# qingxu-thu/INSR-PDE

Hardware: AMD Instinct MI355X
Metric: collocation-points/sec/timestep (incl. ∇/Δ residual + Adam) at 1/2/4/8 GPUs (higher is better)
Workload: dtype fp32

## Files before the change

insr-pde_amd/csrc/jet_x6.hpp:

```cpp
#pragma once
#include "jet_split.hpp"

namespace insr {

typedef short bf16x8 __attribute__((ext_vector_type(8)));
typedef unsigned u32x4 __attribute__((ext_vector_type(4)));
typedef unsigned u32x2 __attribute__((ext_vector_type(2)));
typedef __bf16 bf16x2v __attribute__((ext_vector_type(2)));

__device__ __forceinline__ unsigned pk_bf16(float a, float b) {
  const bf16x2v v = {(__bf16)a, (__bf16)b};
  return __builtin_bit_cast(unsigned, v);
}
__device__ __forceinline__ float bf_lo(unsigned p) { return __builtin_bit_cast(float, p << 16); }
__device__ __forceinline__ float bf_hi(unsigned p) { return __builtin_bit_cast(float, p & 0xffff0000u); }

__device__ __forceinline__ void split3(float a, float b, unsigned& h, unsigned& m, unsigned& l) {
  h = pk_bf16(a, b);
  float ra = a - bf_lo(h), rb = b - bf_hi(h);
  m = pk_bf16(ra, rb);
  ra -= bf_lo(m);
  rb -= bf_hi(m);
  l = pk_bf16(ra, rb);
}

template <int NQ>
constexpr int np_of() { return NQ == 4 ? 2 : NQ; }

template <int NQ>
struct FragQ {
  u32x4 q[np_of<NQ>()];
};

typedef _Float16 f16x2v __attribute__((ext_vector_type(2)));
typedef _Float16 f16x8 __attribute__((ext_vector_type(8)));
__device__ __forceinline__ unsigned pk_f16(float a, float b) {
  const f16x2v v = {(_Float16)a, (_Float16)b};
  return __builtin_bit_cast(unsigned, v);
}
using Frag3 = FragQ<3>;

template <int NQ>
__device__ __forceinline__ void splitq(float a, float b, unsigned (&o)[np_of<NQ>()]) {
  if constexpr (NQ == 4) {
    o[0] = pk_f16(a, b);
    const f16x2v h = __builtin_bit_cast(f16x2v, o[0]);
    o[1] = pk_f16(a - (float)h[0], b - (float)h[1]);
    return;
  }
  o[0] = pk_bf16(a, b);
  if constexpr (NQ > 1) {
    float ra = a - bf_lo(o[0]), rb = b - bf_hi(o[0]);
    o[1] = pk_bf16(ra, rb);
    if constexpr (NQ > 2) {
      ra -= bf_lo(o[1]);
      rb -= bf_hi(o[1]);
      o[2] = pk_bf16(ra, rb);
    }
  }
}

template <int NQ>
__device__ __forceinline__ FragQ<NQ> split_frag(const floatx4& v0, const floatx4& v1) {
  unsigned t[4][np_of<NQ>()];
  splitq<NQ>(v0[0], v0[1], t[0]);
  splitq<NQ>(v0[2], v0[3], t[1]);
  splitq<NQ>(v1[0], v1[1], t[2]);
  splitq<NQ>(v1[2], v1[3], t[3]);
  FragQ<NQ> f;
#pragma unroll
  for (int q = 0; q < np_of<NQ>(); ++q) f.q[q] = u32x4{t[0][q], t[1][q], t[2][q], t[3][q]};
  return f;
}

__device__ __forceinline__ floatx4 mfma_bf(const u32x4& a, const u32x4& b, floatx4 c) {
  return __builtin_amdgcn_mfma_f32_16x16x32_bf16(__builtin_bit_cast(bf16x8, a), __builtin_bit_cast(bf16x8, b), c,
                                                 0, 0, 0);
}

__device__ __forceinline__ floatx4 mfma_h(const u32x4& a, const u32x4& b, floatx4 c) {
  return __builtin_amdgcn_mfma_f32_16x16x32_f16(__builtin_bit_cast(f16x8, a), __builtin_bit_cast(f16x8, b), c, 0, 0, 0);
}

template <int NQ>
__device__ __forceinline__ floatx4 mfma_q(const FragQ<NQ>& a, const FragQ<NQ>& b, floatx4 c) {
  if constexpr (NQ == 4) {
    c = mfma_h(a.q[0], b.q[1], c);
    c = mfma_h(a.q[1], b.q[0], c);
    return mfma_h(a.q[0], b.q[0], c);
  }
  if constexpr (NQ == 3) {
    c = mfma_bf(a.q[1], b.q[1], c);
    c = mfma_bf(a.q[0], b.q[2], c);
    c = mfma_bf(a.q[2], b.q[0], c);
  }
  if constexpr (NQ >= 2) {
    c = mfma_bf(a.q[0], b.q[1], c);
    c = mfma_bf(a.q[1], b.q[0], c);
  }
  return mfma_bf(a.q[0], b.q[0], c);
}

template <int NQ, int PLANE>
__device__ __forceinline__ FragQ<NQ> lds_frag(const unsigned short* p) {
  FragQ<NQ> f;
#pragma unroll
  for (int q = 0; q < np_of<NQ>(); ++q) f.q[q] = *reinterpret_cast<const u32x4*>(p + q * PLANE);
  return f;
}

template <int NQ, int PLANE>
__device__ __forceinline__ void lds_put4(unsigned short* p, float a0, float a1, float a2, float a3) {
  unsigned u0[np_of<NQ>()], u1[np_of<NQ>()];
  splitq<NQ>(a0, a1, u0);
  splitq<NQ>(a2, a3, u1);
#pragma unroll
  for (int q = 0; q < np_of<NQ>(); ++q) *reinterpret_cast<u32x2*>(p + q * PLANE) = u32x2{u0[q], u1[q]};
}

template <int NT>
struct X6Geo {
  static constexpr int W = 16 * NT;
  static constexpr int WV = NT < 8 ? NT : 8;
  static constexpr int RPW = NT / WV;
  static constexpr int KC = NT / 2;
  static constexpr int LDB = W + 8;
  static constexpr int PLANE = 16 * LDB;
  static constexpr int THREADS = 64 * WV;
};

template <int NQ, int NT, int S, int T>
constexpr size_t fwd_x6_lds_bytes() {
  using G = X6Geo<NT>;
  const size_t planes = (size_t)T * S * np_of<NQ>() * G::PLANE * 2 + (NQ == 4 ? (2 * T * 8 + 2 + 8) * sizeof(float) : 0);
  const size_t red = (size_t)G::WV * T * S * 3 * 16 * sizeof(float);
  return planes > red ? planes : red;
}

__device__ __forceinline__ const u32x4* wsp_base(const float* prm, int din, int dout, int L, int W) {
  return reinterpret_cast<const u32x4*>(prm + wsplit_offset(din, dout, L, W));
}
template <int NQ, int NT>
__device__ __forceinline__ FragQ<NQ> wsp_frag(const u32x4* __restrict__ wsp, int L, int o, int j, int rt, int kc,
                                              int lane) {
  constexpr int W = 16 * NT, KC = NT / 2;
  if constexpr (NQ == 4) {
    const u32x4* p = wsp + 2 * wsplit_orient_vecs(L, W) + o * wsplit_f16_vecs(L, W) +
                     ((((long)(j - 1) * NT + rt) * KC + kc) * 2) * 64 + lane;
    FragQ<NQ> f;
    f.q[0] = p[0];
    f.q[1] = p[64];
    return f;
  }
  const u32x4* p = wsp + o * wsplit_orient_vecs(L, W) + ((((long)(j - 1) * NT + rt) * KC + kc) * 3) * 64 + lane;
  FragQ<NQ> f;
#pragma unroll
  for (int q = 0; q < NQ; ++q) f.q[q] = p[q * 64];
  return f;
}

__device__ __forceinline__ int f16_exp_for(float m) {
  if (!(m > 0.f && m <= 3.0e38f)) return 0;
  int k;
  (void)frexpf(m, &k);
  return min(max(15 - k, -100), 100);
}

__device__ __forceinline__ void block_tiles(int b, int N, int T, int nbal, int& tile0, int& cnt) {
  if (nbal > 0) {
    const long tiles = (N + 15) / 16;
    tile0 = (int)(((long)b * tiles) / nbal);
    cnt = (int)((((long)b + 1) * tiles) / nbal) - tile0;
  } else {
    const int tiles = (N + 15) / 16;
    tile0 = b * T;
    cnt = tiles - tile0 < T ? tiles - tile0 : T;
  }
}

template <int NQ, int NT, int S, bool LAP, int T>
__device__ __forceinline__ void fwd_x6_block(const float* __restrict__ x, int N, int din, int dout, int L,
                                             const float* __restrict__ prm, float* __restrict__ y,
                                             float* __restrict__ dy, float* __restrict__ lap,
                                             float* __restrict__ act, const int tile0, const int cnt_rt) {
  using G = X6Geo<NT>;
  constexpr int W = G::W, RPW = G::RPW, LDB = G::LDB, WV = G::WV, PLANE = G::PLANE, KC = G::KC;
  constexpr int NTAN = LAP ? S - 2 : S - 1;
  const int cnt = (T == 3 || T == 5) ? cnt_rt : T;
  extern __shared__ __attribute__((aligned(16))) float lds_f[];
  unsigned short* lds = reinterpret_cast<unsigned short*>(lds_f);
  const int wave = threadIdx.x >> 6, lane = threadIdx.x & 63, g = lane >> 4, c = lane & 15;
  const int ntiles = ((N + 63) / 64) * 4;
  const int rt0 = wave * RPW;
  const u32x4* wsp = wsp_base(prm, din, dout, L, W);
  float* zmx = lds_f + (T * S * np_of<NQ>() * PLANE) / 2;
  float usl[T];
#pragma unroll
  for (int t = 0; t < T; ++t) usl[t] = 1.f / kF16WScale;
  float ust = 1.f / kF16WScale;
  int* tflag = reinterpret_cast<int*>(zmx + 2 * T * 8);
  if constexpr (NQ == 4 && NTAN > 0) {
    if (threadIdx.x < 2) tflag[threadIdx.x] = 0;
  }

  float xv[T][3];
#pragma unroll
  for (int t = 0; t < T; ++t) {
    const int p = (tile0 + t) * 16 + c;
    for (int k = 0; k < 3; ++k) xv[t][k] = (t < cnt && p < N && k < din) ? x[(long)p * din + k] : 0.f;
  }

  floatx4 a[T][RPW][S];
  {
    const float* W0 = prm;
    const float* b0 = prm + (long)W * din;
#pragma unroll
    for (int i = 0; i < RPW; ++i) {
#pragma unroll
      for (int r = 0; r < 4; ++r) {
        const int n = 16 * (rt0 + i) + 4 * g + r;
        const float bn = b0[n];
        float w0[3] = {0.f, 0.f, 0.f};
        for (int k = 0; k < din; ++k) w0[k] = W0[n * din + k];
#pragma unroll
        for (int t = 0; t < T; ++t) {
          float z = bn;
          for (int k = 0; k < din; ++k) z = fmaf(w0[k], xv[t][k], z);
          a[t][i][0][r] = z;
#pragma unroll
          for (int k = 0; k < NTAN; ++k) a[t][i][1 + k][r] = w0[k];
          if constexpr (LAP) a[t][i][S - 1][r] = 0.f;
        }
      }
    }
  }
  for (int j = 0; j <= L; ++j) {
    if (j > 0) {
      const float* Wj = prm + hidden_off(din, W, j);
      const float* bj = Wj + (long)W * W;
#pragma unroll
      for (int i = 0; i < RPW; ++i) {
        const int rt = rt0 + i;
        FragQ<NQ> wf[KC];
#pragma unroll
        for (int kc = 0; kc < KC; ++kc) wf[kc] = wsp_frag<NQ, NT>(wsp, L, 0, j, rt, kc, lane);
        floatx4 bias = *reinterpret_cast<const floatx4*>(bj + 16 * rt + 4 * g);
        if constexpr (NQ == 4) bias *= kF16WScale;
#pragma unroll
        for (int t = 0; t < T; ++t) {
          a[t][i][0] = bias;
#pragma unroll
          for (int s = 1; s < S; ++s) a[t][i][s] = floatx4{0.f, 0.f, 0.f, 0.f};
        }
#pragma unroll
        for (int kc = 0; kc < KC; ++kc) {
#pragma unroll
          for (int t = 0; t < T; ++t) {
            if (t >= cnt) break;
#pragma unroll
            for (int s = 0; s < S; ++s) {
              const unsigned short* pb = lds + (t * S + s) * np_of<NQ>() * PLANE + c * LDB + 32 * kc + 8 * g;
              a[t][i][s] = mfma_q<NQ>(wf[kc], lds_frag<NQ, PLANE>(pb), a[t][i][s]);
            }
          }
        }
        if constexpr (NQ == 4) {
#pragma unroll
          for (int t = 0; t < T; ++t)
#pragma unroll
            for (int s = 0; s < S; ++s)
              a[t][i][s] *= (LAP && s == S - 1) ? usl[t] : (s > 0 ? ust : 1.f / kF16WScale);
        }
      }
    }
    if constexpr (NQ == 4 && LAP) {
      if (j < L) {
#pragma unroll
        for (int t = 0; t < T; ++t) {
          float mt = 0.f;
#pragma unroll
          for (int i = 0; i < RPW; ++i)
#pragma unroll
            for (int r = 0; r < 4; ++r) {
              float t2 = 0.f;
#pragma unroll
              for (int k = 0; k < NTAN; ++k) t2 = fmaf(a[t][i][1 + k][r], a[t][i][1 + k][r], t2);
              mt = fmaxf(mt, fmaf(OMEGA, fabsf(a[t][i][S - 1][r]), OMEGA2 * t2));
            }
          mt = wave_max(mt);
          if (lane == 0) zmx[((j & 1) * T + t) * 8 + wave] = mt;
        }
      }
    }
    auto tan_bound = [&]() -> float {
      float mt = 0.f;
      if (j == 0) {
        for (int n = lane; n < W; n += 64)
          for (int k = 0; k < NTAN; ++k) mt = fmaxf(mt, fabsf(prm[n * din + k]));
      } else {
#pragma unroll
        for (int t = 0; t < T; ++t)
#pragma unroll
          for (int i = 0; i < RPW; ++i)
#pragma unroll
            for (int k = 0; k < NTAN; ++k)
#pragma unroll
              for (int r = 0; r < 4; ++r) mt = fmaxf(mt, fabsf(a[t][i][1 + k][r]));
      }
      return OMEGA * mt;
    };
    bool tbig = false;
    if constexpr (NQ == 4 && NTAN > 0) {
      if (j < L) {
        tbig = __any(tan_bound() >= 32768.f);
        if (j > 0 && tbig && lane == 0) tflag[j & 1] = 1;
      }
    }
    if (j > 0 || (NQ == 4 && LAP)) __syncthreads();
    float sct = 1.f;
    if constexpr (NQ == 4 && NTAN > 0) {
      ust = 1.f / kF16WScale;
      if (j < L) {
        if (j > 0) tbig = __builtin_amdgcn_readfirstlane(tflag[j & 1]) != 0;
        if (tbig) {
          float mt = wave_max(tan_bound());
          if (j > 0) {
            float* tmx = reinterpret_cast<float*>(tflag + 2);
            if (lane == 0) tmx[wave] = mt;
            __syncthreads();
#pragma unroll
            for (int w = 0; w < WV; ++w) mt = fmaxf(mt, tmx[w]);
          }
          const int e = __builtin_amdgcn_readfirstlane(f16_exp_for(mt));
          sct = ldexpf(1.f, e);
          ust = ldexpf(1.f, -e) / kF16WScale;
        }
        if (j > 0 && threadIdx.x == 0) tflag[(j + 1) & 1] = 0;
      }
    }
    if (act) {
      const int ns = l0_rebuilt(j, L) ? 1 : S;
#pragma unroll
      for (int t = 0; t < T; ++t) {
        if (t >= cnt) break;
        float* base = act_base(act, j, ntiles, tile0 + t, S, NT);
#pragma unroll
        for (int i = 0; i < RPW; ++i)
#pragma unroll
          for (int s = 0; s < S; ++s)
            if (s < ns) *reinterpret_cast<floatx4*>(base + ((s * NT + rt0 + i) * 64 + lane) * 4) = a[t][i][s];
      }
    }
#pragma unroll
    for (int t = 0; t < T; ++t) sine_jet<RPW, S, LAP>(a[t]);
    if (j < L) {
      float sll[T];
#pragma unroll
      for (int t = 0; t < T; ++t) {
        sll[t] = 1.f;
        if constexpr (NQ == 4 && LAP) {
          float m = zmx[((j & 1) * T + t) * 8];
#pragma unroll
          for (int w = 1; w < WV; ++w) m = fmaxf(m, zmx[((j & 1) * T + t) * 8 + w]);
          const int e = f16_exp_for(m);
          sll[t] = ldexpf(1.f, e);
          usl[t] = ldexpf(1.f, -e) / kF16WScale;
        }
      }
#pragma unroll
      for (int t = 0; t < T; ++t)
#pragma unroll
        for (int i = 0; i < RPW; ++i)
#pragma unroll
          for (int s = 0; s < S; ++s) {
            unsigned short* pw = lds + (t * S + s) * np_of<NQ>() * PLANE + c * LDB + 16 * (rt0 + i) + 4 * g;
            const float sc = (LAP && s == S - 1) ? sll[t] : (s > 0 ? sct : 1.f);
            lds_put4<NQ, PLANE>(pw, sc * a[t][i][s][0], sc * a[t][i][s][1], sc * a[t][i][s][2], sc * a[t][i][s][3]);
          }
      __syncthreads();
    }
  }
  float* red = lds_f;
  const float* Wo = prm + out_off(din, W, L);
  const float* bo = Wo + (long)dout * W;
  for (int o = 0; o < dout; ++o) {
    float sv[T][S];
#pragma unroll
    for (int t = 0; t < T; ++t)
#pragma unroll
      for (int s = 0; s < S; ++s) sv[t][s] = 0.f;
#pragma unroll
    for (int i = 0; i < RPW; ++i) {
      const floatx4 w4 = *reinterpret_cast<const floatx4*>(Wo + (o * W + 16 * (rt0 + i) + 4 * g));
#pragma unroll
      for (int t = 0; t < T; ++t)
#pragma unroll
        for (int r = 0; r < 4; ++r)
#pragma unroll
          for (int s = 0; s < S; ++s) sv[t][s] = fmaf(w4[r], a[t][i][s][r], sv[t][s]);
    }
#pragma unroll
    for (int t = 0; t < T; ++t)
#pragma unroll
      for (int s = 0; s < S; ++s) {
        float v = sv[t][s];
        v += __shfl_xor(v, 16);
        v += __shfl_xor(v, 32);
        if (g == 0) red[(((wave * T + t) * S + s) * 3 + o) * 16 + c] = v;
      }
  }
  __syncthreads();
  static_assert(T <= 4 * WV, "output stage: one lane group per tile");
  if (wave * 4 + g < cnt) {
    const int t = wave * 4 + g;
    const int p = (tile0 + t) * 16 + c;
    if (p < N) {
      for (int o = 0; o < dout; ++o) {
        float tot[S];
#pragma unroll
        for (int s = 0; s < S; ++s) {
          tot[s] = 0.f;
#pragma unroll
          for (int w = 0; w < WV; ++w) tot[s] += red[(((w * T + t) * S + s) * 3 + o) * 16 + c];
        }
        y[(long)p * dout + o] = tot[0] + bo[o];
        if (dy)
          for (int k = 0; k < NTAN; ++k) dy[((long)p * dout + o) * din + k] = tot[1 + k];
        if constexpr (LAP) {
          if (lap) lap[(long)p * dout + o] = tot[S - 1];
        }
      }
    }
  }
}

template <int NQ, int NT, int S, bool LAP, int T>
constexpr int x6_fwd_min_waves() {
  return ((NT == 8 && (S == 1 || (S == 3 && T <= 2))) || (NQ == 4 && NT == 16 && S == 4 && !LAP && T == 1))
             ? 4
             : 1;
}

template <int NQ, int NT, int S, bool LAP, int T>
__global__ __launch_bounds__(X6Geo<NT>::THREADS, (x6_fwd_min_waves<NQ, NT, S, LAP, T>())) void jet_fwd_x6(
    const float* __restrict__ x, int N, int din, int dout, int L, const float* __restrict__ prm,
    float* __restrict__ y, float* __restrict__ dy, float* __restrict__ lap, float* __restrict__ act, int nbal) {
  int tile0, cnt;
  block_tiles(blockIdx.x, N, T, nbal, tile0, cnt);
  fwd_x6_block<NQ, NT, S, LAP, T>(x, N, din, dout, L, prm, y, dy, lap, act, tile0, cnt);
}

struct FwdJobsX6 {
  InsrJetJob job[kFwdJobs];
  int first[kFwdJobs + 1];
  int small[kFwdJobs];
  int nbal[kFwdJobs];
  int njobs;
};

template <int NQ, int NT, int S, bool LAP, int TA>
constexpr int x6_multi_min_waves() {
  return ((NT == 8 && (S == 1 || S == 3)) || (NQ == 4 && NT == 16 && S == 4 && !LAP && TA == 1)) ? 4 : 1;
}

template <int NQ, int NT, int S, bool LAP, int TA, int TB>
__global__ __launch_bounds__(X6Geo<NT>::THREADS, (x6_multi_min_waves<NQ, NT, S, LAP, TA>())) void jet_fwd_x6_multi(
    const FwdJobsX6 jobs, int din, int dout, int L) {
  const int b = blockIdx.x;
  int k = 0;
#pragma unroll
  for (int q = 1; q < kFwdJobs; ++q) k += (q < jobs.njobs && b >= jobs.first[q]) ? 1 : 0;
  const InsrJetJob& jb = jobs.job[k];
  const int dout_k = jb.d_out > 0 ? jb.d_out : dout;
  if constexpr (TA != TB) {
    if (jobs.small[k]) {
      fwd_x6_block<NQ, NT, S, LAP, TB>(jb.x, (int)jb.n, din, dout_k, L, jb.params, jb.y, jb.dy, jb.lap, jb.act,
                                       (b - jobs.first[k]) * TB, TB);
      return;
    }
  }
  int tile0, cnt;
  block_tiles(b - jobs.first[k], (int)jb.n, TA, jobs.nbal[k], tile0, cnt);
  fwd_x6_block<NQ, NT, S, LAP, TA>(jb.x, (int)jb.n, din, dout_k, L, jb.params, jb.y, jb.dy, jb.lap, jb.act, tile0, cnt);
}

struct FwdMixX6 {
  InsrJetJob job[kFwdJobs];
  int first[kFwdJobs + 1];
  int mode[kFwdJobs];
  float sc[kFwdJobs][3];
  int njobs;
};

constexpr int kMixV = 1, kMixG = 2, kMixL = 4, kMixA = 8;
#ifndef INSR_MIX_ADV_T
#define INSR_MIX_ADV_T 2
#endif
constexpr int kMixAdvT = INSR_MIX_ADV_T;

template <int NQ, int NT, int DIN, int BODIES>
constexpr size_t fwd_mix_lds_bytes() {
  constexpr size_t a = (BODIES & (kMixV | kMixA)) ? fwd_x6_lds_bytes<NQ, NT, 1, 2>() : 0;
  constexpr size_t b = (BODIES & kMixG) ? fwd_x6_lds_bytes<NQ, NT, 1 + DIN, 1>() : 0;
  constexpr size_t c = (DIN <= 2 && (BODIES & kMixL)) ? fwd_x6_lds_bytes<NQ, NT, 2 + DIN, 1>() : 0;
  return a > b ? (a > c ? a : c) : (b > c ? b : c);
}

template <int NQ, int NT, int DIN, int BODIES>
__global__ __launch_bounds__(X6Geo<NT>::THREADS, (BODIES & kMixL) ? 6 : 4) void jet_fwd_x6_mixed(const FwdMixX6 jobs,
                                                                                              int dout, int L) {
  const int b = blockIdx.x;
  int k = 0;
#pragma unroll
  for (int q = 1; q < kFwdJobs; ++q) k += (q < jobs.njobs && b >= jobs.first[q]) ? 1 : 0;
  const InsrJetJob& jb = jobs.job[k];
  const int dk = jb.d_out > 0 ? jb.d_out : dout;
  const int lb = b - jobs.first[k];
  int tile0, cnt;
  switch (jobs.mode[k]) {
    case INSR_MODE_VALUE:
      if constexpr ((BODIES & kMixV) != 0) {
        block_tiles(lb, (int)jb.n, 2, 0, tile0, cnt);
        fwd_x6_block<NQ, NT, 1, false, 2>(jb.x, (int)jb.n, DIN, dk, L, jb.params, jb.y, jb.dy, jb.lap, jb.act, tile0,
                                          cnt);
      }
      break;
    case INSR_MODE_GRAD:
      if constexpr ((BODIES & kMixG) != 0)
        fwd_x6_block<NQ, NT, 1 + DIN, false, 1>(jb.x, (int)jb.n, DIN, dk, L, jb.params, jb.y, jb.dy, jb.lap, jb.act,
                                                lb, 1);
      break;
    case INSR_MODE_LAP:
      if constexpr (DIN <= 2 && (BODIES & kMixL) != 0)
        fwd_x6_block<NQ, NT, 2 + DIN, true, 1>(jb.x, (int)jb.n, DIN, dk, L, jb.params, jb.y, jb.dy, jb.lap, jb.act,
                                               lb, 1);
      break;
    case INSR_MIX_ADVECT: {
      if constexpr ((BODIES & kMixA) == 0) break;
      const int n = (int)jb.n;
      block_tiles(lb, n, kMixAdvT, 0, tile0, cnt);
      float* up = jb.dy;
      float* foot = jb.lap;
      fwd_x6_block<NQ, NT, 1, false, kMixAdvT>(jb.x, n, DIN, dk, L, jb.params, up, nullptr, nullptr, nullptr, tile0,
                                               cnt);
      __builtin_amdgcn_fence(__ATOMIC_SEQ_CST, "workgroup");
      __syncthreads();
      const float a = -jobs.sc[k][0], lo = jobs.sc[k][1], hi = jobs.sc[k][2];
      for (int i = threadIdx.x; i < cnt * 16 * DIN; i += blockDim.x) {
        const long p = (long)tile0 * 16 + i / DIN;
        const int kk = i % DIN;
        if (p < n) foot[p * DIN + kk] = fminf(fmaxf(fmaf(a, up[p * dk + kk], jb.x[p * DIN + kk]), lo), hi);
      }
      __builtin_amdgcn_fence(__ATOMIC_SEQ_CST, "workgroup");
      __syncthreads();
      fwd_x6_block<NQ, NT, 1, false, kMixAdvT>(foot, n, DIN, dk, L, jb.params, jb.y, nullptr, nullptr, nullptr, tile0,
                                               cnt);
      break;
    }
    default:
      break;
  }
}

template <int NQ, int NT, int DIN, int BODIES>
int launch_fwd_x6_mixed_t(const InsrJetJob* jobs, const int* modes, const float* scalars, int njobs, int dout, int L,
                          hipStream_t st) {
  constexpr size_t lds = fwd_mix_lds_bytes<NQ, NT, DIN, BODIES>();
  if constexpr (lds > kLdsMax) {
    return INSR_EINVAL;
  } else {
    if (njobs < 1 || njobs > kFwdJobs) return INSR_EINVAL;
    static const bool attr_set = ((void)hipFuncSetAttribute((const void*)jet_fwd_x6_mixed<NQ, NT, DIN, BODIES>,
                                hipFuncAttributeMaxDynamicSharedMemorySize, (int)lds), true);
    (void)attr_set;
    FwdMixX6 pk{};
    int nb = 0;
    for (int k = 0; k < njobs; ++k) {
      if (modes[k] == INSR_MODE_LAP && DIN > 2) return INSR_EINVAL;
      pk.job[k] = jobs[k];
      pk.mode[k] = modes[k];
      for (int q = 0; q < 3; ++q) pk.sc[k][q] = scalars ? scalars[3 * k + q] : 0.f;
      pk.first[k] = nb;
      const long tiles = (jobs[k].n + 15) / 16;
      nb += (int)(modes[k] == INSR_MODE_VALUE ? (tiles + 1) / 2
                                              : (modes[k] == INSR_MIX_ADVECT ? (tiles + kMixAdvT - 1) / kMixAdvT : tiles));
    }
    pk.first[njobs] = nb;
    pk.njobs = njobs;
    if (nb == 0) return 0;
    hipLaunchKernelGGL((jet_fwd_x6_mixed<NQ, NT, DIN, BODIES>), dim3(nb), dim3(X6Geo<NT>::THREADS), lds, st, pk, dout,
                       L);
    return (int)hipGetLastError();
  }
}

template <int NQ, int NT, int S, bool LAP, int T>
int launch_fwd_x6_multi_t(const InsrJetJob* jobs, const int* small, const int* nbal, int njobs, int din, int dout,
                          int L, hipStream_t st) {
  constexpr int TB = T <= 2 ? T : 1;
  constexpr size_t lds = fwd_x6_lds_bytes<NQ, NT, S, T>();
  if constexpr (lds > kLdsMax) {
    return INSR_EINVAL;
  } else {
    if (njobs < 1 || njobs > kFwdJobs) return INSR_EINVAL;
    static const bool attr_set = ((void)hipFuncSetAttribute((const void*)jet_fwd_x6_multi<NQ, NT, S, LAP, T, TB>,
                                hipFuncAttributeMaxDynamicSharedMemorySize, (int)lds), true);
    (void)attr_set;
    FwdJobsX6 pk{};
    int nb = 0, m = 0;
    for (int pass = 0; pass < 2; ++pass)
      for (int k = 0; k < njobs; ++k) {
        const int sm = (T != TB && small && small[k]) ? 1 : 0;
        if (sm != 1 - pass) continue;
        pk.job[m] = jobs[k];
        pk.small[m] = sm;
        pk.nbal[m] = sm ? 0 : (nbal ? nbal[k] : 0);
        pk.first[m] = nb;
        const int t = sm ? TB : T;
        nb += pk.nbal[m] > 0 ? pk.nbal[m] : (int)(((jobs[k].n + 15) / 16 + t - 1) / t);
        ++m;
      }
    pk.first[njobs] = nb;
    pk.njobs = njobs;
    if (nb == 0) return 0;
    hipLaunchKernelGGL((jet_fwd_x6_multi<NQ, NT, S, LAP, T, TB>), dim3(nb), dim3(X6Geo<NT>::THREADS), lds, st, pk, din,
                       dout, L);
    return (int)hipGetLastError();
  }
}

template <int NQ, int NT, int S, bool LAP, int T>
int launch_fwd_x6_t(const float* x, int N, int din, int dout, int L, const float* prm, float* y, float* dy,
                    float* lap, float* act, int nbal, hipStream_t st) {
  constexpr size_t lds = fwd_x6_lds_bytes<NQ, NT, S, T>();
  if constexpr (lds > kLdsMax) {
    return INSR_EINVAL;
  } else {
    const int nb = ((N + 15) / 16 + T - 1) / T;
    static const bool attr_set = ((void)hipFuncSetAttribute((const void*)jet_fwd_x6<NQ, NT, S, LAP, T>, hipFuncAttributeMaxDynamicSharedMemorySize,
                                (int)lds), true);
    (void)attr_set;
    if (N < 0) {
      int occ = 0;
      (void)hipOccupancyMaxActiveBlocksPerMultiprocessor(&occ, (const void*)jet_fwd_x6<NQ, NT, S, LAP, T>, X6Geo<NT>::THREADS, lds);
      return occ;
    }
    hipLaunchKernelGGL((jet_fwd_x6<NQ, NT, S, LAP, T>), dim3(nbal > 0 ? nbal : nb), dim3(X6Geo<NT>::THREADS), lds, st,
                       x, N, din, dout, L, prm, y, dy, lap, act, nbal);
    return (int)hipGetLastError();
  }
}

}

namespace insr {

template <int S, bool LAP>
__device__ __forceinline__ floatx4 h_from_regs(int s, const floatx4 (&zd)[S - 1], const floatx4& sn,
                                               const floatx4& cs) {
  constexpr int NTAN = LAP ? S - 2 : S - 1;
  if (s == 0) return sn;
  floatx4 out;
  if (LAP && s == S - 1) {
#pragma unroll
    for (int r = 0; r < 4; ++r) {
      float t2 = 0.f;
#pragma unroll
      for (int i = 0; i < NTAN; ++i) t2 = fmaf(zd[i][r], zd[i][r], t2);
      out[r] = OMEGA * cs[r] * zd[s - 1][r] - OMEGA2 * sn[r] * t2;
    }
  } else {
#pragma unroll
    for (int r = 0; r < 4; ++r) out[r] = OMEGA * cs[r] * zd[s - 1][r];
  }
  return out;
}

#define X6_SCHED_FENCE() __builtin_amdgcn_sched_barrier(0)

__device__ __forceinline__ float dpp_xor1(float v) {
  return __builtin_bit_cast(float, __builtin_amdgcn_update_dpp(0, __builtin_bit_cast(int, v), 0xB1, 0xF, 0xF, false));
}
__device__ __forceinline__ float dpp_xor2(float v) {
  return __builtin_bit_cast(float, __builtin_amdgcn_update_dpp(0, __builtin_bit_cast(int, v), 0x4E, 0xF, 0xF, false));
}
__device__ __forceinline__ floatx4 quad_transpose(const floatx4& v, int c) {
  const bool o1 = c & 1, o2 = c & 2;
  const float s0 = dpp_xor1(o1 ? v[0] : v[1]), s1 = dpp_xor1(o1 ? v[2] : v[3]);
  const floatx4 a = {o1 ? s0 : v[0], o1 ? v[1] : s0, o1 ? s1 : v[2], o1 ? v[3] : s1};
  const float t0 = dpp_xor2(o2 ? a[0] : a[2]), t1 = dpp_xor2(o2 ? a[1] : a[3]);
  return floatx4{o2 ? t0 : a[0], o2 ? t1 : a[1], o2 ? a[2] : t0, o2 ? a[3] : t1};
}

typedef short v4s __attribute__((ext_vector_type(4)));
__device__ __forceinline__ v4s ds_read_tr16(const unsigned short* p) {
  return __builtin_amdgcn_ds_read_tr16_b64_v4i16((__attribute__((address_space(3))) v4s*)(p));
}

template <int NQ, int PLANE>
__device__ __forceinline__ void put_neuron_major(unsigned short* P, const floatx4& v, int row0, int c) {
  const floatx4 tv = quad_transpose(v, c);
  lds_put4<NQ, PLANE>(P + (row0 + (c & 3)) * 16 + (c & ~3), tv[0], tv[1], tv[2], tv[3]);
}

template <int NQ, int NT>
struct X6BwdGeo {
  using G = X6Geo<NT>;
  static constexpr int W = G::W;
  static constexpr int ZROW = G::LDB;
  static constexpr int ZPLANE = 16 * ZROW;
  static constexpr int ZSET = np_of<NQ>() * ZPLANE + 32;
  static constexpr int HPLANE = W * 16;
  static constexpr int HSET = np_of<NQ>() * HPLANE;
  static constexpr size_t SET_BYTES = (size_t)(ZSET + HSET) * 2;
};

template <int NQ, int NT, int S, int T>
constexpr int x6_bwd_sg() {
  constexpr size_t set = X6BwdGeo<NQ, NT>::SET_BYTES;
  if ((size_t)T * S * set <= kLdsMax) return S;
  if (S % 2 == 0 && (size_t)T * (S / 2) * set <= kLdsMax) return S / 2;
  return 1;
}

template <int S, int T>
constexpr size_t bwd_x6_seed_floats() {
  return S == 1 ? (size_t)T * 48 + 8 * INSR_SEED_MAX : 0;
}
template <int NQ, int NT, int S, int T>
constexpr size_t bwd_x6_lds_bytes() {
  return (size_t)T * x6_bwd_sg<NQ, NT, S, T>() * X6BwdGeo<NQ, NT>::SET_BYTES + 2 * 5 * 8 * sizeof(float) +
         bwd_x6_seed_floats<S, T>() * sizeof(float);
}

template <int NQ, int NT, int S, bool LAP, int T>
__global__ __launch_bounds__(X6Geo<NT>::THREADS) void jet_bwd_x6(const BwdJobsX6 J, int din, int dout, int L,
                                                                  const float* __restrict__ prm,
                                                                  float* __restrict__ part, long P) {
  using G = X6Geo<NT>;
  using BG = X6BwdGeo<NQ, NT>;
  constexpr int W = G::W, RPW = G::RPW, KC = G::KC;
  constexpr int LDB = BG::ZROW, ZPLANE = BG::ZPLANE, ZSET = BG::ZSET, HPLANE = BG::HPLANE, HSET = BG::HSET;
  constexpr int NTAN = LAP ? S - 2 : S - 1;
  constexpr int SG = x6_bwd_sg<NQ, NT, S, T>();
  constexpr int NG = S / SG;
  constexpr int NSET = T * SG;
  constexpr int NCH = (NSET + 1) / 2;
  static_assert(S % SG == 0, "stream groups");
  static_assert(NG == 1 || RPW * NT <= 16, "dW accumulators across groups");
  extern __shared__ __attribute__((aligned(16))) float lds_f[];
  unsigned short* Z = reinterpret_cast<unsigned short*>(lds_f);
  unsigned short* H = Z + NSET * ZSET;
  float* zred = lds_f + NSET * (ZSET + HSET) / 2;
  const int wave = threadIdx.x >> 6, lane = threadIdx.x & 63, g = lane >> 4, c = lane & 15;
  const int b = blockIdx.x;
  int jk = 0;
#pragma unroll
  for (int q = 1; q < kBwdJobs; ++q) jk += (q < J.njobs && b >= J.first[q]) ? 1 : 0;
  const float* __restrict__ x = J.x[jk];
  const float* __restrict__ act = J.act[jk];
  const float* __restrict__ gy = J.gy[jk];
  const float* __restrict__ gdy = J.gdy[jk];
  const float* __restrict__ glap = J.glap[jk];
  const int N = J.n[jk];
  const int ntiles = ((N + 63) / 64) * 4;
  int tile0, cnt_rt;
  block_tiles(b - J.first[jk], N, T, J.nbal[jk], tile0, cnt_rt);
  const int cnt = (T == 3 || T == 5) ? cnt_rt : T;
  auto tt = [&](int t) { return tile0 + (t < cnt_rt ? t : 0); };
  const int rt0 = wave * RPW;
  float* mypart = part + (long)blockIdx.x * P;

  float* sseed = zred + 2 * 5 * 8;
  constexpr bool kSeed1 = S == 1 && T * 48 <= G::THREADS;
  SeedOps sop{0.f, 0.f, 0.f, 0.f, -1};
  float sgy = 0.f;
  if constexpr (kSeed1) {
    if (J.seeds.nt) {
      const int i = threadIdx.x, t = i / 48, o = (i / 16) % 3, p = (tile0 + t) * 16 + (i & 15);
      if (i < T * 48 && t < cnt && p < N && o < dout) {
        const long e = (long)p * dout + o;
        if (gy)
          sgy = gy[e];
        else
          sop = seed_gather(J.seeds, jk, INSR_SEED_VALUE, e);
      }
    }
  }
  auto seed_stage = [&]() {
    if constexpr (S == 1) {
      if (J.seeds.nt) {
        float* swq = sseed + T * 48;
        float sq[INSR_SEED_MAX] = {0.f, 0.f, 0.f, 0.f};
        if constexpr (kSeed1) {
          if (threadIdx.x < T * 48) sseed[threadIdx.x] = gy ? sgy : seed_finish(J.seeds, sop, sq);
        } else {
          for (int i = threadIdx.x; i < T * 48; i += G::THREADS) {
            const int t = i / 48, o = (i / 16) % 3, p = (tile0 + t) * 16 + (i & 15);
            float v = 0.f;
            if (t < cnt && p < N && o < dout) {
              const long e = (long)p * dout + o;
              v = gy ? gy[e] : seed_adjoint(J.seeds, jk, INSR_SEED_VALUE, e, true, sq);
            }
            sseed[i] = v;
          }
        }
#pragma unroll
        for (int q = 0; q < INSR_SEED_MAX; ++q) {
          float v = sq[q];
          for (int off = 32; off > 0; off >>= 1) v += __shfl_xor(v, off);
          if (lane == 0) swq[wave * INSR_SEED_MAX + q] = v;
        }
        __syncthreads();
        if (threadIdx.x == 0) {
          floatx4 r = floatx4{0.f, 0.f, 0.f, 0.f};
          for (int w = 0; w < G::THREADS / 64; ++w)
#pragma unroll
            for (int q = 0; q < INSR_SEED_MAX; ++q) r[q] += swq[w * INSR_SEED_MAX + q];
          *reinterpret_cast<floatx4*>(J.seeds.lpart + (long)blockIdx.x * INSR_SEED_MAX) = r;
        }
      }
    }
  };
  auto adjoint = [&](int t, int s, int o) -> float {
    const int p = (tile0 + t) * 16 + c;
    if constexpr (S == 1)
      if (J.seeds.nt) return sseed[(t * 3 + o) * 16 + c];
    if (t >= cnt || p >= N) return 0.f;
    if (s == 0) return gy ? gy[(long)p * dout + o] : 0.f;
    if (LAP && s == S - 1) return glap ? glap[(long)p * dout + o] : 0.f;
    return gdy ? gdy[((long)p * dout + o) * din + (s - 1)] : 0.f;
  };

  auto load_sc = [&](int layer, floatx4(&s_)[T][RPW], floatx4(&c_)[T][RPW]) {
    floatx4 z[T][RPW];
    float amax = 0.f;
#pragma unroll
    for (int t = 0; t < T; ++t) {
      const float* base = act_base(act, layer, ntiles, tt(t), S, NT);
#pragma unroll
      for (int i = 0; i < RPW; ++i) {
        z[t][i] = *reinterpret_cast<const floatx4*>(base + ((rt0 + i) * 64 + lane) * 4);
#pragma unroll
        for (int r = 0; r < 4; ++r) amax = fmaxf(amax, fabsf(OMEGA * z[t][i][r]));
      }
    }
    const bool big = wave_any_big(amax);
#pragma unroll
    for (int t = 0; t < T; ++t)
#pragma unroll
      for (int i = 0; i < RPW; ++i)
#pragma unroll
        for (int r = 0; r < 4; ++r) {
          float sv, cv;
          if (big)
            sincosf(OMEGA * z[t][i][r], &sv, &cv);
          else
            sincos_fast(OMEGA * z[t][i][r], sv, cv);
          s_[t][i][r] = sv;
          c_[t][i][r] = cv;
        }
  };

  floatx4 sn[T][RPW], cs[T][RPW];
  load_sc(L, sn, cs);
  seed_stage();
  const float* Wo = prm + out_off(din, W, L);
  const long wo_off = out_off(din, W, L);
  floatx4 hb[T][RPW][S];
#pragma unroll
  for (int t = 0; t < T; ++t)
#pragma unroll
    for (int i = 0; i < RPW; ++i)
#pragma unroll
      for (int s = 0; s < S; ++s) hb[t][i][s] = floatx4{0.f, 0.f, 0.f, 0.f};
  for (int o = 0; o < dout; ++o) {
    float ga[T][S];
#pragma unroll
    for (int t = 0; t < T; ++t)
#pragma unroll
      for (int s = 0; s < S; ++s) ga[t][s] = adjoint(t, s, o);
#pragma unroll
    for (int i = 0; i < RPW; ++i) {
      const int rt = rt0 + i;
      const floatx4 w4 = *reinterpret_cast<const floatx4*>(Wo + (o * W + 16 * rt + 4 * g));
      floatx4 acc4 = floatx4{0.f, 0.f, 0.f, 0.f};
#pragma unroll
      for (int t = 0; t < T; ++t) {
        const float* baseL = act_base(act, L, ntiles, tt(t), S, NT);
#pragma unroll
        for (int s = 0; s < S; ++s) {
          const floatx4 hs = h_stream<NT, S, LAP>(baseL, s, rt, lane, sn[t][i], cs[t][i]);
#pragma unroll
          for (int r = 0; r < 4; ++r) {
            acc4[r] = fmaf(ga[t][s], hs[r], acc4[r]);
            hb[t][i][s][r] = fmaf(w4[r], ga[t][s], hb[t][i][s][r]);
          }
        }
      }
#pragma unroll
      for (int r = 0; r < 4; ++r) {
        const float v = sum16(acc4[r]);
        if (c == 0) mypart[wo_off + (long)o * W + 16 * rt + 4 * g + r] = v;
      }
    }
    if (wave == 0) {
      float v = 0.f;
#pragma unroll
      for (int t = 0; t < T; ++t) v += (g == 0) ? ga[t][0] : 0.f;
      v = sum16(v);
      if (lane == 0) mypart[wo_off + (long)dout * W + o] = v;
    }
  }

#ifndef X6_KZ_MAX
#define X6_KZ_MAX 3
#endif
  constexpr bool KZ = S > 1 && T * RPW * (S - 1) <= X6_KZ_MAX;
  constexpr int ZK = KZ ? S - 1 : 1;
  floatx4 zk[KZ ? T : 1][KZ ? RPW : 1][ZK];
  auto load_zk = [&](int layer) {
    if constexpr (KZ) {
#pragma unroll
      for (int t = 0; t < T; ++t) {
        const float* base = act_base(act, layer, ntiles, tt(t), S, NT);
        const bool l0 = l0_rebuilt(layer, L);
#pragma unroll
        for (int i = 0; i < RPW; ++i)
#pragma unroll
          for (int s = 1; s < S; ++s) zk[t][i][s - 1] = load_zs<NT, S, LAP>(base, s, rt0 + i, lane, l0, prm, din);
      }
    }
  };
  load_zk(L);
  const u32x4* wsp = wsp_base(prm, din, dout, L, W);
  for (int j = L; j >= 0; --j) {
    INSR_STAMP(L - j, 0);
#pragma unroll
    for (int t = 0; t < T; ++t) {
      const float* basej = act_base(act, j, ntiles, tt(t), S, NT);
#pragma unroll
      for (int i = 0; i < RPW; ++i) {
        if constexpr (KZ) {
          floatx4 zs[S];
          zs[0] = floatx4{0.f, 0.f, 0.f, 0.f};
#pragma unroll
          for (int s = 1; s < S; ++s) zs[s] = zk[t][i][s - 1];
          sine_rev<S, LAP>(hb[t][i], zs, sn[t][i], cs[t][i]);
        } else {
          floatx4 zs[S];
#pragma unroll
          for (int s = 0; s < S; ++s)
            zs[s] = (s == 0) ? floatx4{0.f, 0.f, 0.f, 0.f}
                             : load_zs<NT, S, LAP>(basej, s, rt0 + i, lane, l0_rebuilt(j, L), prm, din);
          sine_rev<S, LAP>(hb[t][i], zs, sn[t][i], cs[t][i]);
        }
      }
    }
    const long boff = (j == 0) ? (long)W * din : hidden_off(din, W, j) + (long)W * W;
#pragma unroll
    for (int i = 0; i < RPW; ++i)
#pragma unroll
      for (int r = 0; r < 4; ++r) {
        float v = 0.f;
#pragma unroll
        for (int t = 0; t < T; ++t) v += hb[t][i][0][r];
        v = sum16(v);
        if (c == 0) mypart[boff + 16 * (rt0 + i) + 4 * g + r] = v;
      }
    if (j == 0) {
#pragma unroll
      for (int i = 0; i < RPW; ++i)
        for (int k = 0; k < din; ++k)
#pragma unroll
          for (int r = 0; r < 4; ++r) {
            float v = 0.f;
#pragma unroll
            for (int t = 0; t < T; ++t) {
              const int p = (tile0 + t) * 16 + c;
              const float xk = (t < cnt && p < N) ? x[(long)p * din + k] : 0.f;
              v = fmaf(hb[t][i][0][r], xk, v);
              if (k < NTAN) v += hb[t][i][1 + k][r];
            }
            v = sum16(v);
            if (c == 0) mypart[(long)(16 * (rt0 + i) + 4 * g + r) * din + k] = v;
          }
      break;
    }
    INSR_STAMP(L - j, 1);
    if constexpr (NQ == 4) {
      float mv = 0.f, mt = 0.f, ml = 0.f;
#pragma unroll
      for (int t = 0; t < T; ++t)
#pragma unroll
        for (int i = 0; i < RPW; ++i)
#pragma unroll
          for (int s = 0; s < S; ++s)
#pragma unroll
            for (int r = 0; r < 4; ++r) {
              if (LAP && s == S - 1)
                ml = fmaxf(ml, fabsf(hb[t][i][s][r]));
              else if (s == 0)
                mv = fmaxf(mv, fabsf(hb[t][i][s][r]));
              else
                mt = fmaxf(mt, fabsf(hb[t][i][s][r]));
            }
      mv = wave_max(mv);
      if constexpr (S > 1) mt = wave_max(mt);
      if constexpr (LAP) ml = wave_max(ml);
      if (lane == 0) {
        zred[((j & 1) * 5) * 8 + wave] = mv;
        zred[((j & 1) * 5 + 1) * 8 + wave] = ml;
        zred[((j & 1) * 5 + 3) * 8 + wave] = mt;
      }
    }
    FragQ<NQ> wt[RPW][KC];
    if constexpr (NG == 1) {
#pragma unroll
      for (int i = 0; i < RPW; ++i)
#pragma unroll
        for (int kc = 0; kc < KC; ++kc) wt[i][kc] = wsp_frag<NQ, NT>(wsp, L, 1, j, rt0 + i, kc, lane);
    }
    floatx4 snp[T][RPW], csp[T][RPW];
    load_sc(j - 1, snp, csp);
    load_zk(j - 1);
    if constexpr (NQ == 4 && S > 1) {
      float hl = 0.f, htb = 0.f;
#pragma unroll
      for (int t = 0; t < T; ++t) {
        const float* basep = act_base(act, j - 1, ntiles, tt(t), S, NT);
#pragma unroll
        for (int i = 0; i < RPW; ++i) {
          floatx4 zd[S - 1];
#pragma unroll
          for (int s = 1; s < S; ++s) {
            if constexpr (KZ)
              zd[s - 1] = zk[t][i][s - 1];
            else
              zd[s - 1] = load_zs<NT, S, LAP>(basep, s, rt0 + i, lane, l0_rebuilt(j - 1, L), prm, din);
          }
#pragma unroll
          for (int r = 0; r < 4; ++r) {
            float t2 = 0.f;
#pragma unroll
            for (int k = 0; k < NTAN; ++k) {
              t2 = fmaf(zd[k][r], zd[k][r], t2);
              htb = fmaxf(htb, fabsf(zd[k][r]));
            }
            if constexpr (LAP) hl = fmaxf(hl, fmaf(OMEGA, fabsf(zd[S - 2][r]), OMEGA2 * t2));
          }
        }
      }
      if constexpr (LAP) hl = wave_max(hl);
      htb = wave_max(htb) * OMEGA;
      if (lane == 0) {
        zred[((j & 1) * 5 + 2) * 8 + wave] = hl;
        zred[((j & 1) * 5 + 4) * 8 + wave] = htb;
      }
    }
    floatx4 dacc[RPW][NT];
#pragma unroll
    for (int i = 0; i < RPW; ++i)
#pragma unroll
      for (int ct = 0; ct < NT; ++ct) dacc[i][ct] = floatx4{0.f, 0.f, 0.f, 0.f};
    floatx4 nh[T][RPW][S];
    float zsc = 1.f, zun = 1.f, zll = 1.f, hll = 1.f, ztl = 1.f, htl = 1.f;
#pragma unroll
    for (int gi = 0; gi < NG; ++gi) {
      const int s0 = gi * SG;
      INSR_STAMP(L - j, 2);
      __syncthreads();
      INSR_STAMP(L - j, 3);
      if constexpr (NQ == 4) {
        if (gi == 0) {
          const float* zr = zred + (j & 1) * 5 * 8;
          float mv = zr[0], ml = zr[8], mh = zr[16], mt = zr[24], mht = zr[32];
#pragma unroll
          for (int w = 1; w < G::WV; ++w) {
            mv = fmaxf(mv, zr[w]);
            ml = fmaxf(ml, zr[8 + w]);
            mh = fmaxf(mh, zr[16 + w]);
            mt = fmaxf(mt, zr[24 + w]);
            mht = fmaxf(mht, zr[32 + w]);
          }
          if constexpr (LAP) {
            hll = ldexpf(1.f, f16_exp_for(mh));
            zll = 1.f / hll;
          }
          if constexpr (S > 1) {
            htl = ldexpf(1.f, mht >= 32768.f ? f16_exp_for(mht) : 0);
            ztl = 1.f / htl;
          }
          const int e = f16_exp_for(fmaxf(mv, fmaxf(mt * ztl, ml * zll)));
          zsc = ldexpf(1.f, e);
          zun = ldexpf(1.f, -e);
        }
      }
#pragma unroll
      for (int t = 0; t < T; ++t) {
        const float* basep = act_base(act, j - 1, ntiles, tt(t), S, NT);
#pragma unroll
        for (int i = 0; i < RPW; ++i)
#pragma unroll
          for (int sl = 0; sl < SG; ++sl) {
            const int s = s0 + sl;
            const int u = t * SG + sl;
            const int col = 16 * (rt0 + i) + 4 * g;
            const bool lq = NQ == 4 && LAP && s == S - 1;
            const bool tq = NQ == 4 && s > 0 && !lq;
            const float fl = lq ? zll : (tq ? ztl : 1.f);
            lds_put4<NQ, ZPLANE>(Z + u * ZSET + c * LDB + col, (hb[t][i][s][0] * zsc) * fl,
                                 (hb[t][i][s][1] * zsc) * fl, (hb[t][i][s][2] * zsc) * fl,
                                 (hb[t][i][s][3] * zsc) * fl);
            floatx4 hs;
            if constexpr (KZ) {
              hs = h_from_regs<S, LAP>(s, zk[t][i], snp[t][i], csp[t][i]);
            } else {
              hs = h_stream<NT, S, LAP>(basep, s, rt0 + i, lane, snp[t][i], csp[t][i], l0_rebuilt(j - 1, L), prm,
                                        din);
            }
            if (lq) hs *= hll;
            if (tq) hs *= htl;
            put_neuron_major<NQ, HPLANE>(H + u * HSET, hs, col, c);
          }
      }
      INSR_STAMP(L - j, 4);
      __syncthreads();
      INSR_STAMP(L - j, 5);
#pragma unroll
      for (int ch = 0; ch < NCH; ++ch) {
        if (2 * ch >= cnt * SG) break;
        const int u = 2 * ch + (g >> 1);
        const bool live = u < cnt * SG;
        const int p0 = 8 * (g & 1);
#pragma unroll
        for (int i = 0; i < RPW; ++i) {
          FragQ<NQ> af;
          {
            const unsigned short* pa =
                Z + (live ? u : 0) * ZSET + (p0 + (c >> 2)) * LDB + 16 * (rt0 + i) + 4 * (c & 3);
#pragma unroll
            for (int q = 0; q < np_of<NQ>(); ++q) {
              const v4s lo = ds_read_tr16(pa + q * ZPLANE);
              const v4s hi = ds_read_tr16(pa + q * ZPLANE + 4 * LDB);
              const u32x2 wl = __builtin_bit_cast(u32x2, lo), wh = __builtin_bit_cast(u32x2, hi);
              af.q[q] = live ? u32x4{wl[0], wl[1], wh[0], wh[1]} : u32x4{0u, 0u, 0u, 0u};
            }
          }
#pragma unroll
          for (int ct = 0; ct < NT; ++ct) {
            const FragQ<NQ> bf = lds_frag<NQ, HPLANE>(H + (live ? u : 0) * HSET + (16 * ct + c) * 16 + p0);
            dacc[i][ct] = mfma_q<NQ>(af, bf, dacc[i][ct]);
            X6_SCHED_FENCE();
          }
        }
      }
      if constexpr (NG == 1) {
        float* dW = mypart + hidden_off(din, W, j);
#pragma unroll
        for (int i = 0; i < RPW; ++i)
#pragma unroll
          for (int ct = 0; ct < NT; ++ct)
#pragma unroll
            for (int r = 0; r < 4; ++r) dW[(16 * (rt0 + i) + 4 * g + r) * W + 16 * ct + c] = dacc[i][ct][r] * zun;
      }
      INSR_STAMP(L - j, 6);
      if constexpr (NG > 1) {
#pragma unroll
        for (int i = 0; i < RPW; ++i)
#pragma unroll
          for (int kc = 0; kc < KC; ++kc) wt[i][kc] = wsp_frag<NQ, NT>(wsp, L, 1, j, rt0 + i, kc, lane);
      }
#pragma unroll
      for (int t = 0; t < T; ++t)
#pragma unroll
        for (int sl = 0; sl < SG; ++sl) {
          const int s = s0 + sl;
          const int u = t * SG + sl;
#pragma unroll
          for (int i = 0; i < RPW; ++i) nh[t][i][s] = floatx4{0.f, 0.f, 0.f, 0.f};
          if (t >= cnt) continue;
#pragma unroll
          for (int kc = 0; kc < KC; ++kc) {
            const FragQ<NQ> bf = lds_frag<NQ, ZPLANE>(Z + u * ZSET + c * LDB + 32 * kc + 8 * g);
#pragma unroll
            for (int i = 0; i < RPW; ++i) nh[t][i][s] = mfma_q<NQ>(wt[i][kc], bf, nh[t][i][s]);
            X6_SCHED_FENCE();
          }
        }
    }
    INSR_STAMP(L - j, 7);
    if constexpr (NG > 1) {
      float* dW = mypart + hidden_off(din, W, j);
#pragma unroll
      for (int i = 0; i < RPW; ++i)
#pragma unroll
        for (int ct = 0; ct < NT; ++ct)
#pragma unroll
          for (int r = 0; r < 4; ++r) dW[(16 * (rt0 + i) + 4 * g + r) * W + 16 * ct + c] = dacc[i][ct][r] * zun;
    }
#pragma unroll
    for (int t = 0; t < T; ++t)
#pragma unroll
      for (int i = 0; i < RPW; ++i) {
        sn[t][i] = snp[t][i];
        cs[t][i] = csp[t][i];
#pragma unroll
        for (int s = 0; s < S; ++s)
          hb[t][i][s] = (NQ == 4) ? (nh[t][i][s] * zun) *
                                        (((LAP && s == S - 1) ? hll : (s > 0 ? htl : 1.f)) / kF16WScale)
                                  : nh[t][i][s];
      }
  }
}

template <int NQ, int NT, int S, bool LAP, int T>
int launch_bwd_x6_t(const BwdJobsX6* J, int din, int dout, int L, const float* prm, float* part, long P,
                    hipStream_t st) {
  constexpr size_t lds = bwd_x6_lds_bytes<NQ, NT, S, T>();
  if constexpr (lds > kLdsMax || NT > 8) {
    return INSR_EINVAL;
  } else {
    static const bool attr_set = ((void)hipFuncSetAttribute((const void*)jet_bwd_x6<NQ, NT, S, LAP, T>,
                                hipFuncAttributeMaxDynamicSharedMemorySize, (int)lds), true);
    (void)attr_set;
    if (!J) {
      int occ = 0;
      (void)hipOccupancyMaxActiveBlocksPerMultiprocessor(&occ, (const void*)jet_bwd_x6<NQ, NT, S, LAP, T>, X6Geo<NT>::THREADS, lds);
      return occ;
    }
    if (J->njobs < 1 || J->njobs > kBwdJobs) return INSR_EINVAL;
    const int nb = J->first[J->njobs];
    if (nb <= 0) return 0;
    hipLaunchKernelGGL((jet_bwd_x6<NQ, NT, S, LAP, T>), dim3(nb), dim3(X6Geo<NT>::THREADS), lds, st, *J, din, dout, L,
                       prm, part, P);
    return (int)hipGetLastError();
  }
}

}
```

Baseline: 113.9 million.

## Track fp16 tangent scale per tile and raise launch bounds for DIN=2

```diff
diff --git a/insr-pde_amd/csrc/jet_x6.hpp b/insr-pde_amd/csrc/jet_x6.hpp
--- a/insr-pde_amd/csrc/jet_x6.hpp
+++ b/insr-pde_amd/csrc/jet_x6.hpp
@@ -132,7 +132,8 @@
 template <int NQ, int NT, int S, int T>
 constexpr size_t fwd_x6_lds_bytes() {
   using G = X6Geo<NT>;
-  const size_t planes = (size_t)T * S * np_of<NQ>() * G::PLANE * 2 + (NQ == 4 ? (2 * T * 8 + 2 + 8) * sizeof(float) : 0);
+  const size_t planes =
+      (size_t)T * S * np_of<NQ>() * G::PLANE * 2 + (NQ == 4 ? (2 * T * 8 + 2 * T + 8 * T) * sizeof(float) : 0);
   const size_t red = (size_t)G::WV * T * S * 3 * 16 * sizeof(float);
   return planes > red ? planes : red;
 }
@@ -197,10 +198,12 @@
   float usl[T];
 #pragma unroll
   for (int t = 0; t < T; ++t) usl[t] = 1.f / kF16WScale;
-  float ust = 1.f / kF16WScale;
+  float ust[T];
+#pragma unroll
+  for (int t = 0; t < T; ++t) ust[t] = 1.f / kF16WScale;
   int* tflag = reinterpret_cast<int*>(zmx + 2 * T * 8);
   if constexpr (NQ == 4 && NTAN > 0) {
-    if (threadIdx.x < 2) tflag[threadIdx.x] = 0;
+    if (threadIdx.x < 2 * T) tflag[threadIdx.x] = 0;
   }
 
   float xv[T][3];
@@ -269,7 +272,7 @@
           for (int t = 0; t < T; ++t)
 #pragma unroll
             for (int s = 0; s < S; ++s)
-              a[t][i][s] *= (LAP && s == S - 1) ? usl[t] : (s > 0 ? ust : 1.f / kF16WScale);
+              a[t][i][s] *= (LAP && s == S - 1) ? usl[t] : (s > 0 ? ust[t] : 1.f / kF16WScale);
         }
       }
     }
@@ -287,55 +290,76 @@
               for (int k = 0; k < NTAN; ++k) t2 = fmaf(a[t][i][1 + k][r], a[t][i][1 + k][r], t2);
               mt = fmaxf(mt, fmaf(OMEGA, fabsf(a[t][i][S - 1][r]), OMEGA2 * t2));
             }
-          mt = wave_max(mt);
+          mt = wave_max_nn(mt);
           if (lane == 0) zmx[((j & 1) * T + t) * 8 + wave] = mt;
         }
       }
     }
-    auto tan_bound = [&]() -> float {
+    auto tan_bound = [&](int t) -> float {
       float mt = 0.f;
       if (j == 0) {
         for (int n = lane; n < W; n += 64)
           for (int k = 0; k < NTAN; ++k) mt = fmaxf(mt, fabsf(prm[n * din + k]));
       } else {
 #pragma unroll
-        for (int t = 0; t < T; ++t)
-#pragma unroll
-          for (int i = 0; i < RPW; ++i)
-#pragma unroll
-            for (int k = 0; k < NTAN; ++k)
-#pragma unroll
-              for (int r = 0; r < 4; ++r) mt = fmaxf(mt, fabsf(a[t][i][1 + k][r]));
+        for (int i = 0; i < RPW; ++i)
+#pragma unroll
+          for (int k = 0; k < NTAN; ++k)
+#pragma unroll
+            for (int r = 0; r < 4; ++r) mt = fmaxf(mt, fabsf(a[t][i][1 + k][r]));
       }
       return OMEGA * mt;
     };
-    bool tbig = false;
+    bool tbig[T], tany = false;
+#pragma unroll
+    for (int t = 0; t < T; ++t) tbig[t] = false;
     if constexpr (NQ == 4 && NTAN > 0) {
       if (j < L) {
-        tbig = __any(tan_bound() >= 32768.f);
-        if (j > 0 && tbig && lane == 0) tflag[j & 1] = 1;
+#pragma unroll
+        for (int t = 0; t < T; ++t) {
+          tbig[t] = (j == 0 && t > 0) ? tbig[0] : __any(tan_bound(t) >= 32768.f);
+          if (j > 0 && tbig[t] && lane == 0) tflag[(j & 1) * T + t] = 1;
+        }
       }
     }
     if (j > 0 || (NQ == 4 && LAP)) __syncthreads();
-    float sct = 1.f;
+    float sct[T];
+#pragma unroll
+    for (int t = 0; t < T; ++t) sct[t] = 1.f;
     if constexpr (NQ == 4 && NTAN > 0) {
-      ust = 1.f / kF16WScale;
+#pragma unroll
+      for (int t = 0; t < T; ++t) ust[t] = 1.f / kF16WScale;
       if (j < L) {
-        if (j > 0) tbig = __builtin_amdgcn_readfirstlane(tflag[j & 1]) != 0;
-        if (tbig) {
-          float mt = wave_max(tan_bound());
-          if (j > 0) {
-            float* tmx = reinterpret_cast<float*>(tflag + 2);
-            if (lane == 0) tmx[wave] = mt;
-            __syncthreads();
-#pragma unroll
-            for (int w = 0; w < WV; ++w) mt = fmaxf(mt, tmx[w]);
-          }
-          const int e = __builtin_amdgcn_readfirstlane(f16_exp_for(mt));
-          sct = ldexpf(1.f, e);
-          ust = ldexpf(1.f, -e) / kF16WScale;
-        }
-        if (j > 0 && threadIdx.x == 0) tflag[(j + 1) & 1] = 0;
+#pragma unroll
+        for (int t = 0; t < T; ++t) {
+          if (j > 0) tbig[t] = __builtin_amdgcn_readfirstlane(tflag[(j & 1) * T + t]) != 0;
+          tany = tany || tbig[t];
+        }
+        if (tany) {
+          float mt[T];
+          float* tmx = reinterpret_cast<float*>(tflag + 2 * T);
+#pragma unroll
+          for (int t = 0; t < T; ++t) {
+            mt[t] = 0.f;
+            if (tbig[t]) {
+              mt[t] = (j == 0 && t > 0) ? mt[0] : wave_max_nn(tan_bound(t));
+              if (j > 0 && lane == 0) tmx[t * 8 + wave] = mt[t];
+            }
+          }
+          if (j > 0) __syncthreads();
+#pragma unroll
+          for (int t = 0; t < T; ++t) {
+            if (!tbig[t]) continue;
+            if (j > 0) {
+#pragma unroll
+              for (int w = 0; w < WV; ++w) mt[t] = fmaxf(mt[t], tmx[t * 8 + w]);
+            }
+            const int e = __builtin_amdgcn_readfirstlane(f16_exp_for(mt[t]));
+            sct[t] = ldexpf(1.f, e);
+            ust[t] = ldexpf(1.f, -e) / kF16WScale;
+          }
+        }
+        if (j > 0 && threadIdx.x < T) tflag[((j + 1) & 1) * T + threadIdx.x] = 0;
       }
     }
     if (act) {
@@ -374,7 +398,7 @@
 #pragma unroll
           for (int s = 0; s < S; ++s) {
             unsigned short* pw = lds + (t * S + s) * np_of<NQ>() * PLANE + c * LDB + 16 * (rt0 + i) + 4 * g;
-            const float sc = (LAP && s == S - 1) ? sll[t] : (s > 0 ? sct : 1.f);
+            const float sc = (LAP && s == S - 1) ? sll[t] : (s > 0 ? sct[t] : 1.f);
             lds_put4<NQ, PLANE>(pw, sc * a[t][i][s][0], sc * a[t][i][s][1], sc * a[t][i][s][2], sc * a[t][i][s][3]);
           }
       __syncthreads();
@@ -507,8 +531,13 @@
 }
 
 template <int NQ, int NT, int DIN, int BODIES>
-__global__ __launch_bounds__(X6Geo<NT>::THREADS, (BODIES & kMixL) ? 6 : 4) void jet_fwd_x6_mixed(const FwdMixX6 jobs,
-                                                                                              int dout, int L) {
+constexpr int x6_mixed_min_waves() {
+  return (BODIES & kMixL) ? 6 : ((NQ == 4 && DIN == 2) ? 8 : 4);
+}
+
+template <int NQ, int NT, int DIN, int BODIES>
+__global__ __launch_bounds__(X6Geo<NT>::THREADS, (x6_mixed_min_waves<NQ, NT, DIN, BODIES>())) void jet_fwd_x6_mixed(
+    const FwdMixX6 jobs, int dout, int L) {
   const int b = blockIdx.x;
   int k = 0;
 #pragma unroll
```

After: 114.3 million, median of 4. No clear change (+0.4%).
